# HpWang-whu/RoReg

Hardware: AMD Instinct MI355X
Metric: pair-registrations/sec (higher is better)
Workload: dtype f32 (every f32 operand enters the fp16 matrix cores as hi + lo fp16 under a per-keypoint power-of-two block scale: <= 22 significant bits relative to a CONSERVATIVE per-keypoint bound -- measured on the extractor: the bound sits 2^2..2^6 above the keypoint's true coefficient maximum (config.f16x2_sc

## Files before the change

### include/roreg_hip.h

```cpp
#ifndef ROREG_HIP_H
#define ROREG_HIP_H

#include <stdint.h>
#include <stddef.h>

#ifdef __cplusplus
extern "C" {
#endif

#define ROREG_ABI_VERSION 6
int roreg_abi_version(void);
const char *roreg_last_error(void);

int roreg_set_group_tables(const int32_t *P_host, const int32_t *Nei_host, const double *R_host);

size_t roreg_group_conv_packed_size(int Cin, int Cout, int KS);
int roreg_group_conv_pack_weights(const float *W_host , int Cin, int Cout, int KS,
                                  float *wpack_host );
size_t roreg_group_conv_workspace_size(int B, int Cin, int Cout, int Lin, int Lout, int KS);
int roreg_group_conv(const float *x, const float *wpack, const float *bias,
                     const float *bn_scale, const float *bn_shift, const float *residual,
                     float *out, const int32_t *gather,
                     int B, int Cin, int Cout, int Lin, int Lout, int KS,
                     float *workspace, size_t workspace_floats, void *stream);

int roreg_group_conv_split(const float *x, const void *wsplit, const float *bias, const float *bn_scale, const float *bn_shift,
                           float *out, const int32_t *gather,
                           const int32_t *lds_order , int lds_stride,
                           int B, int Cin, int Cout, int Lin, int Lout, int KS, void *stream);

int roreg_dense_split(const float *x, const void *wsplit, const float *bias, const float *scale, const float *shift,
                      const float *residual, int residual_stride, float *out, int B, int K, int O, void *stream);

int roreg_group_conv_f16x2(const float *x, const void *wsplit2, int w_exp, const float *bias, const float *bn_scale, const float *bn_shift,
                           float act_smax, float act_tmax, const float *in_rowmax_dev, float *out, float *out_rowmax_dev,
                           const int32_t *gather, const int32_t *lds_order , int lds_stride,
                           int B, int Cin, int Cout, int Lin, int Lout, int KS, void *stream);
int roreg_dense_f16x2(const float *x, const void *wsplit2, int w_exp, const float *bias, const float *scale, const float *shift,
                      float act_smax, float act_tmax, const float *in_rowmax_dev, const float *residual, int residual_stride, float *out,
                      float *out_rowmax_dev, int B, int K, int O, void *stream);
int roreg_group_conv_f16x2_packed(const uint32_t *x_words, const void *wsplit2, int w_exp, const float *bias, const float *in_bound_dev,
                                  float *out, float *out_rowmax_dev, const int32_t *gather, const int32_t *lds_order, int lds_stride,
                                  int B, int Cin, int Cout, int Lin, int Lout, int KS, void *stream);

int roreg_gf_finalize(const float *eqv_raw, void *eqv, int eqv_bf16 ,
                      float *inv, int B, void *stream);

int roreg_det_score(const float *enc, float *scores, int B, void *stream);

int roreg_inv_descriptor(const void *eqv, int eqv_bf16 , float *inv, int N,
                         void *stream);

int roreg_nn_search(const float *src, const int64_t *src_rows, int m,
                    const float *tgt, const int64_t *tgt_rows, int n, int F,
                    int64_t *idx_out, float *dist_out, uint64_t *scratch, void *stream);

int roreg_nn_search_ex(const float *src, const int64_t *src_rows, int m,
                       const float *tgt, const int64_t *tgt_rows, int n, int F, int squared,
                       int64_t *idx_out, float *dist_out, uint64_t *scratch, void *stream);

int roreg_pdist(const float *A, int m, const float *B, int n, int F, int squared, float *out, void *stream);

typedef struct {
    const float *desc0, *desc1;
    const int64_t *rows0, *rows1;
    int32_t m0, m1;
} roreg_match_task;
size_t roreg_mutual_match_batch_workspace(int n_tasks, int max_m);
int roreg_mutual_match_batch(const roreg_match_task *tasks_dev, int n_tasks, int max_m, int64_t *match_out, int32_t *counts_out,
                             void *workspace, size_t workspace_bytes, void *stream);

size_t roreg_knn_search_workspace(int m, int n);
int roreg_knn_search(const float *src, int m, const float *tgt, int n, int F, int k,
                     int64_t *idx_out, void *workspace , size_t workspace_bytes, void *stream);

int roreg_knn_search_ex(const float *src, int m, const float *tgt, int n, int F, int k, int squared, int64_t *idx_out, float *dist_out,
                        void *workspace, size_t workspace_bytes, void *stream);

size_t roreg_knn_search_seg_workspace(long long m_total, int n_seg, int max_m, int max_n);
int roreg_knn_search_seg(const float *src, const float *tgt, const int32_t *seg_src, const int32_t *seg_tgt, int n_seg, long long m_total,
                         int max_m, int max_n, int F, int k, int64_t *idx_out, void *workspace, size_t workspace_bytes, void *stream);

int roreg_mutual_matches(const int64_t *nn01, const int64_t *nn10, int m, int n ,
                         const int64_t *sample0, const int64_t *sample1,
                         int64_t *match_out, int32_t *count_out, void *stream);

int roreg_des2r(const float *feats1, const int64_t *rows1, const float *feats0, const int64_t *rows0,
                int M, int64_t *idx_out, float *cor_out, void *stream);

int roreg_group_corr(const float *perm_feats, const int64_t *perm_rows, const float *bcast_feats, const int64_t *bcast_rows,
                     int M, int transpose_table, int64_t *idx_out, float *cor_out, void *stream);

int roreg_group_corr_mfma(const float *perm_feats, const int64_t *perm_rows, const float *bcast_feats, const int64_t *bcast_rows, int M,
                          int transpose_table, float *cor_out, void *stream);

int roreg_set_des2r_tables(int transpose_table , const uint8_t *ia_host,
                           const uint8_t *ib_host, const uint8_t *cnt_host, const float *NT_host);
int roreg_group_corr_irrep(const float *perm_coefs, const int64_t *perm_rows, const float *bcast_coefs, const int64_t *bcast_rows, int M,
                           int transpose_table, float *cor_out, void *stream);
int roreg_des2r_irrep(const float *coef1, const int64_t *rows1, const float *coef0, const int64_t *rows0, const void *feats1,
                      const void *feats0, int feat_bf16, int M, int64_t *idx_out, void *stream);
int roreg_des2r_recheck_count(int reset, int32_t *count_out);
int roreg_feat_coefs(const void *x, int x_bf16, float *out, int B, int C, int split, void *stream);

int roreg_et_gather(const void *before0, const void *before1, const void *after0, const void *after1,
                    int feat_bf16 ,
                    const int64_t *rows0, const int64_t *rows1, const int64_t *pre_idx, int M,
                    float *x_out, void *stream);

int roreg_quat_to_trans(const float *q, const int64_t *anchor, const double *keys0, const int64_t *rows0,
                        const double *keys1, const int64_t *rows1, int M,
                        double *Trans_out, float *quat_out, void *stream);

int roreg_ransac_score(const double *k0, const double *k1, const double *w, int w_f32, int M,
                       const double *Trans, const int64_t *hyp_rows, int H, double ird,
                       double *overlap_out, int32_t *best_out, uint8_t *mask_out, void *stream);

int roreg_refine(const double *k0, const double *k1, const double *w, int w_f32, int M,
                 const double *T_in, int t_in_stride ,
                 const double *Trans, const int64_t *hyp_rows, const int32_t *best,
                 double dist, double *T_out, double *stats_out ,
                 void *stream);

typedef struct {
    const void *before0, *before1, *after0, *after1;
    const double *keys0, *keys1;
    const int64_t *matches;
    const int64_t *sel;
    int32_t n, pad_;
    int64_t off;
    const float *coef0, *coef1;
} roreg_lt_task;
int roreg_lt_prepare_batch(const roreg_lt_task *tasks_dev, int n_tasks, int max_n, int flags, int64_t *dr_out, float *x_out,
                           const float *bn_scale , const float *bn_shift, float *x_bound_out , void *stream);
int roreg_lt_finish_batch(const roreg_lt_task *tasks_dev, int n_tasks, int max_n, const float *q_all, const int64_t *dr_all,
                          double *Trans_out, void *stream);
int roreg_role_max(const void *before, const void *after, int feat_bf16, const float *bn_scale , const float *bn_shift, float *out,
                   int N, void *stream);
int roreg_row_bound_roles(const void *x_spatial, int x_bf16, float *bound_out, const float *role_scale, const float *role_shift, float *role_out, int B,
                          void *stream);
int roreg_inv_descriptor_roles(const void *eqv, int eqv_bf16, float *inv, const float *role_scale, const float *role_shift, float *role_out, int N,
                               void *stream);
int roreg_lt_prepare_rows(const roreg_lt_task *tasks_dev, const float *const *roles_dev, int n_tasks, int max_n, int flags, int64_t *dr_out,
                          uint64_t *rows_out, float *x_bound_out, void *stream);

typedef struct {
    const double *keys0, *keys1;
    const int64_t *matches;
    const double *w;
    const double *Trans;
    const int64_t *hyp_rows;
    int32_t M, H;
    int64_t koff;
// ... 258 lines not shown
```

### roreg_amd/_abi.py

```python
import ctypes
from ctypes import c_int, c_void_p, c_size_t, c_double, c_float, c_char_p

import numpy as np

ABI_VERSION = 6

_P = c_void_p
PROTOTYPES = {
    'roreg_abi_version': (c_int, []),
    'roreg_last_error': (c_char_p, []),
    'roreg_set_group_tables': (c_int, [_P, _P, _P]),
    'roreg_group_conv_packed_size': (c_size_t, [c_int, c_int, c_int]),
    'roreg_group_conv_pack_weights': (c_int, [_P, c_int, c_int, c_int, _P]),
    'roreg_group_conv_workspace_size': (c_size_t, [c_int, c_int, c_int, c_int, c_int, c_int]),
    'roreg_group_conv': (c_int, [_P, _P, _P, _P, _P, _P, _P, _P, c_int, c_int, c_int, c_int, c_int, c_int, _P, c_size_t, _P]),
    'roreg_group_conv_split': (c_int, [_P, _P, _P, _P, _P, _P, _P, _P, c_int, c_int, c_int, c_int, c_int, c_int, c_int, _P]),
    'roreg_group_conv_f16x2': (c_int, [_P, _P, c_int, _P, _P, _P, c_float, c_float, _P, _P, _P, _P, _P, c_int, c_int, c_int, c_int, c_int, c_int, c_int, _P]),
    'roreg_group_conv_f16x2_packed': (c_int, [_P, _P, c_int, _P, _P, _P, _P, _P, _P, c_int, c_int, c_int, c_int, c_int, c_int, c_int, _P]),
    'roreg_dense_f16x2': (c_int, [_P, _P, c_int, _P, _P, _P, c_float, c_float, _P, _P, c_int, _P, _P, c_int, c_int, c_int, _P]),
    'roreg_dense_split': (c_int, [_P, _P, _P, _P, _P, _P, c_int, _P, c_int, c_int, c_int, _P]),
    'roreg_gf_finalize': (c_int, [_P, _P, c_int, _P, c_int, _P]),
    'roreg_det_score': (c_int, [_P, _P, c_int, _P]),
    'roreg_inv_descriptor': (c_int, [_P, c_int, _P, c_int, _P]),
    'roreg_nn_search': (c_int, [_P, _P, c_int, _P, _P, c_int, c_int, _P, _P, _P, _P]),
    'roreg_nn_search_ex': (c_int, [_P, _P, c_int, _P, _P, c_int, c_int, c_int, _P, _P, _P, _P]),
    'roreg_pdist': (c_int, [_P, c_int, _P, c_int, c_int, c_int, _P, _P]),
    'roreg_knn_search_workspace': (c_size_t, [c_int, c_int]),
    'roreg_knn_search': (c_int, [_P, c_int, _P, c_int, c_int, c_int, _P, _P, c_size_t, _P]),
    'roreg_knn_search_ex': (c_int, [_P, c_int, _P, c_int, c_int, c_int, c_int, _P, _P, _P, c_size_t, _P]),
    'roreg_knn_search_seg_workspace': (c_size_t, [ctypes.c_longlong, c_int, c_int, c_int]),
    'roreg_knn_search_seg': (c_int, [_P, _P, _P, _P, c_int, ctypes.c_longlong, c_int, c_int, c_int, c_int, _P, _P, c_size_t, _P]),
    'roreg_mutual_matches': (c_int, [_P, _P, c_int, c_int, _P, _P, _P, _P, _P]),
    'roreg_mutual_match_batch_workspace': (c_size_t, [c_int, c_int]),
    'roreg_mutual_match_batch': (c_int, [_P, c_int, c_int, _P, _P, _P, c_size_t, _P]),
    'roreg_des2r': (c_int, [_P, _P, _P, _P, c_int, _P, _P, _P]),
    'roreg_set_des2r_tables': (c_int, [c_int, _P, _P, _P, _P]),
    'roreg_group_corr_irrep': (c_int, [_P, _P, _P, _P, c_int, c_int, _P, _P]),
    'roreg_group_corr_mfma': (c_int, [_P, _P, _P, _P, c_int, c_int, _P, _P]),
    'roreg_des2r_irrep': (c_int, [_P, _P, _P, _P, _P, _P, c_int, c_int, _P, _P]),
    'roreg_des2r_recheck_count': (c_int, [c_int, _P]),
    'roreg_feat_coefs': (c_int, [_P, c_int, _P, c_int, c_int, c_int, _P]),
    'roreg_et_gather': (c_int, [_P, _P, _P, _P, c_int, _P, _P, _P, c_int, _P, _P]),
    'roreg_quat_to_trans': (c_int, [_P, _P, _P, _P, _P, _P, c_int, _P, _P, _P]),
    'roreg_ransac_score': (c_int, [_P, _P, _P, c_int, c_int, _P, _P, c_int, c_double, _P, _P, _P, _P]),
    'roreg_refine': (c_int, [_P, _P, _P, c_int, c_int, _P, c_int, _P, _P, _P, c_double, _P, _P, _P]),
    'roreg_lt_prepare_batch': (c_int, [_P, c_int, c_int, c_int, _P, _P, _P, _P, _P, _P]),
    'roreg_lt_finish_batch': (c_int, [_P, c_int, c_int, _P, _P, _P, _P]),
    'roreg_role_max': (c_int, [_P, _P, c_int, _P, _P, _P, c_int, _P]),
    'roreg_row_bound_roles': (c_int, [_P, c_int, _P, _P, _P, _P, c_int, _P]),
    'roreg_inv_descriptor_roles': (c_int, [_P, c_int, _P, _P, _P, _P, c_int, _P]),
    'roreg_lt_prepare_rows': (c_int, [_P, _P, c_int, c_int, c_int, _P, _P, _P, _P]),
    'roreg_ransac_batch_workspace': (c_size_t, [c_int, ctypes.c_longlong, c_int]),
    'roreg_ransac_batch': (c_int, [_P, c_int, ctypes.c_longlong, c_int, c_int, c_double, c_int, _P, _P, _P, _P, _P, _P, c_size_t, _P]),
    'roreg_refine_batch': (c_int, [_P, _P, c_int, ctypes.c_longlong, _P, ctypes.c_double, c_int, _P, _P, _P, _P]),
    'roreg_yohoc_draw': (c_int, [_P, ctypes.c_longlong, _P, _P, c_int, c_int, _P, _P, _P, _P]),
    'roreg_gather_rows_batch': (c_int, [_P, c_int, c_int, c_int, _P]),
    'roreg_gather_rows_f64': (c_int, [_P, _P, c_int, c_int, _P, _P]),
    'roreg_group_corr': (c_int, [_P, _P, _P, _P, c_int, c_int, _P, _P, _P]),
    'roreg_topk_dot_workspace_size': (c_size_t, [c_int, c_int, c_int]),
    'roreg_topk_dot': (c_int, [_P, c_int, _P, c_int, c_int, _P, _P, _P, c_size_t, _P, _P, c_int, c_int, c_int, _P]),
    'roreg_context_colmax': (c_int, [_P, c_int, _P, c_int, c_int, _P, _P, _P]),
    'roreg_sinkhorn_batch_workspace_size': (c_size_t, [c_int, c_int, c_int, ctypes.c_longlong, ctypes.c_longlong]),
    'roreg_sinkhorn_batch_consts': (c_int, [_P, _P, c_int, _P]),
    'roreg_sinkhorn_batch': (c_int, [_P, _P, _P, _P, _P, _P, _P, c_int, c_float, c_int, _P, _P, _P, _P, _P, c_size_t, _P]),
    'roreg_sinkhorn_batch2_workspace_size': (c_size_t, [c_int, c_int, c_int, ctypes.c_longlong, ctypes.c_longlong]),
    'roreg_sinkhorn_batch2': (c_int, [_P, _P, _P, _P, _P, _P, _P, c_int, c_float, c_int, _P, _P, _P, _P, _P, c_size_t, c_int, _P]),
    'roreg_sinkhorn_batch3_workspace_size': (c_size_t, [c_int, c_int, c_int, ctypes.c_longlong, ctypes.c_longlong, c_int, c_int]),
    'roreg_sinkhorn_batch3': (c_int, [_P, _P, _P, _P, _P, _P, _P, c_int, c_float, c_int, _P, _P, _P, _P, _P, c_size_t, c_int, _P, _P]),
    'roreg_write_files': (c_int, [_P, _P, _P, _P, _P, c_int, c_int]),
    'roreg_yohoc_draw_many': (c_int, [_P, c_int, _P, _P, c_int, c_int, _P, _P, _P, c_int]),
    'roreg_mlp_head_workspace': (c_size_t, [c_int, c_int, c_int]),
    'roreg_mlp_head': (c_int, [_P, _P, _P, _P, _P, c_int, c_int, c_int, c_int, _P, _P, c_int, _P, _P, _P, _P, _P, c_int, c_int, c_float, _P, _P, _P]),
    'roreg_sinkhorn_early_exit': (c_int, [c_int]),
    'roreg_sinkhorn_iteration_stats': (c_int, [_P, _P, c_int, _P]),
    'roreg_linear': (c_int, [_P, c_int, c_int, _P, _P, c_int, _P, _P]),
    'roreg_linear_mfma': (c_int, [_P, c_int, c_int, _P, _P, c_int, _P, _P]),
    'roreg_linear_path': (c_int, [c_int]),
    'roreg_linear_cat3': (c_int, [_P, _P, _P, _P, c_int, c_int, _P, _P, c_int, _P, _P]),
    'roreg_gemm_persistent': (c_int, [c_int]),
    'roreg_gemm_thin': (c_int, [c_int]),
    'roreg_gf_finish_route': (c_int, [c_int]),
    'roreg_irrep_gemm_f16x2_rows': (c_int, [_P, _P, _P, _P, c_int, c_int, c_int, _P]),
    'roreg_gf_finish': (c_int, [_P, _P, _P, _P, _P, _P, _P, _P, _P, c_int, _P]),
    'roreg_instnorm_stats': (c_int, [_P, c_int, c_int, c_float, _P, _P, _P, c_int, c_int, _P]),
    'roreg_mlp_tail': (c_int, [_P, c_int, c_int, _P, _P, _P, _P, _P, c_int, c_int, _P]),
    'roreg_mlp_tail_mfma': (c_int, [_P, c_int, c_int, _P, _P, _P, _P, _P, c_int, c_int, _P]),
    'roreg_knn_attention': (c_int, [_P, _P, _P, _P, c_int, c_int, c_int, c_int, _P, _P]),
    'roreg_rm_elementwise': (c_int, [c_int, _P, _P, _P, _P, c_int, c_int, c_int, _P, _P, _P]),
    'roreg_sinkhorn_workspace_size': (c_size_t, [c_int, c_int]),
    'roreg_sinkhorn': (c_int, [_P, c_int, _P, c_int, c_float, c_int, _P, _P, _P, _P, _P, _P, c_size_t, _P]),
    'roreg_icp_grid_size': (c_size_t, [_P, _P, c_int, c_double, _P, _P]),
    'roreg_icp_grid_build': (c_int, [_P, _P, _P, _P, c_size_t, _P]),
    'roreg_icp_batch_workspace': (c_size_t, [c_int, ctypes.c_longlong]),
    'roreg_icp_batch': (c_int, [_P, c_int, _P, c_int, ctypes.c_longlong, c_double, c_int, c_double, c_double, _P, _P, _P, _P, _P, _P, _P, _P, c_size_t, _P]),
    'roreg_icp_normals': (c_int, [_P, c_double, c_int, _P, _P]),
    'roreg_icp_plane_batch_workspace': (c_size_t, [c_int, ctypes.c_longlong]),
    'roreg_icp_plane_batch': (c_int, [_P, c_int, _P, c_int, ctypes.c_longlong, c_double, c_int, c_double, c_double, _P, _P, _P, _P, _P, _P, _P, _P, c_size_t, _P]),
    'roreg_icp_gicp_batch_workspace': (c_size_t, [c_int, ctypes.c_longlong]),
    'roreg_icp_gicp_batch': (c_int, [_P, c_int, _P, c_int, ctypes.c_longlong, c_double, c_int, c_double, c_double, _P, _P, _P, _P, _P, _P, _P, _P, c_size_t, _P]),
    'roreg_icp_eval_workspace': (c_size_t, [c_int, ctypes.c_longlong]),
    'roreg_icp_eval_batch': (c_int, [_P, c_int, _P, c_int, ctypes.c_longlong, c_double, _P, _P, _P, _P, _P, c_size_t, _P]),
    'roreg_voxel_workspace': (c_size_t, [c_int]),
    'roreg_voxel_downsample': (c_int, [_P, c_int, c_double, _P, _P, _P, _P, _P, _P, _P, c_size_t, _P]),
    'roreg_pg_workspace': (c_size_t, [_P, c_int]),
    'roreg_pg_optimize_batch': (c_int, [_P, _P, c_int, _P, _P, _P, _P, _P, _P, _P, _P, _P, _P, _P, c_int, c_int, _P, _P, _P, _P, _P, _P, _P, _P, _P, _P, _P, c_size_t, _P]),
    'roreg_sparse_map_workspace': (c_size_t, [c_int]),
    'roreg_sparse_stride_map': (c_int, [_P, c_int, c_int, _P, c_int, _P, _P, _P, _P, _P, c_size_t, _P]),
    'roreg_sparse_kernel_map': (c_int, [_P, c_int, _P, c_int, c_int, c_int, _P, _P, _P, c_size_t, _P]),
    'roreg_sparse_conv': (c_int, [_P, c_int, c_int, c_int, _P, c_int, c_int, _P, c_int, _P, _P, _P, c_int, c_int, _P, c_int, _P]),
    'roreg_sparse_l2norm': (c_int, [_P, c_int, c_int, _P, _P]),
    'roreg_group_feature_assemble': (c_int, [_P, c_int, c_int, _P, _P, c_int, c_int, c_int, _P, c_int, _P, _P]),
    'roreg_sc2_workspace': (c_size_t, [ctypes.c_longlong, ctypes.c_longlong, ctypes.c_longlong, _P]),
    'roreg_sc2_hypotheses_batch': (c_int, [_P, c_int, ctypes.c_longlong, ctypes.c_longlong, ctypes.c_longlong, c_int, c_int, c_double, c_int, _P, _P, _P, _P, c_size_t, _P]),
    'roreg_fpfh_spfh_workspace': (c_size_t, [c_int]),
    'roreg_fpfh_features_workspace': (c_size_t, [c_int]),
    'roreg_fpfh_orient': (c_int, [_P, c_int, _P, _P, _P, _P]),
    'roreg_fpfh_spfh': (c_int, [_P, c_int, _P, c_double, _P, _P, _P, c_size_t, _P]),
# ... 53 lines not shown
```

### roreg_amd/csrc/mfma_match.hip

```cpp
#include "common.h"
#include "primitives.h"

#pragma clang fp contract(off)

namespace {

struct MatchTask {
    const float *desc0, *desc1;
    const int64_t *rows0, *rows1;
    int32_t m0, m1;
};

constexpr int F = 32, TILE = 128, LP = 36;
constexpr float PAD_NORM = 1e30f;

struct WS {
    float *G;
    float *N;
    unsigned *AM;
    unsigned long long *PK;
    unsigned *MX;
};
__host__ __device__ inline size_t ws_task_bytes(int P) { return (size_t)2 * P * (F * 4 + 4 + 4 + 8) + 64; }
__device__ __forceinline__ WS ws_of(char *base, int task, int P) {
    char *p = base + (size_t)task * ws_task_bytes(P);
    WS w;
    w.PK = reinterpret_cast<unsigned long long *>(p); p += (size_t)2 * P * 8;
    w.G = reinterpret_cast<float *>(p); p += (size_t)2 * P * F * 4;
    w.N = reinterpret_cast<float *>(p); p += (size_t)2 * P * 4;
    w.AM = reinterpret_cast<unsigned *>(p); p += (size_t)2 * P * 4;
    w.MX = reinterpret_cast<unsigned *>(p);
    return w;
}

__device__ __forceinline__ unsigned f2o(float x) { const unsigned b = __float_as_uint(x); return b ^ ((b >> 31) ? 0xffffffffu : 0x80000000u); }
__device__ __forceinline__ float o2f(unsigned k) { return __uint_as_float(k ^ ((k >> 31) ? 0x80000000u : 0xffffffffu)); }

__global__ __launch_bounds__(256) void mm_prepare_kernel(const MatchTask *__restrict__ tasks, int P, char *__restrict__ wsb) {
    const int task = blockIdx.z >> 1, side = blockIdx.z & 1;
    const MatchTask t = tasks[task];
    const WS w = ws_of(wsb, task, P);
    const float *desc = side ? t.desc1 : t.desc0;
    const int64_t *rows = side ? t.rows1 : t.rows0;
    const int m = side ? t.m1 : t.m0;
    const int j = blockIdx.x * 8 + (threadIdx.x >> 5), f = threadIdx.x & 31;
    if (blockIdx.x == 0 && threadIdx.x == 0) w.MX[side] = 0u;
    if (j >= P) return;
    float v = 0.f;
    if (j < m) v = desc[(size_t)(rows ? rows[j] : (int64_t)j) * F + f];
    w.G[((size_t)side * P + j) * F + f] = v;
    float s = v * v;
#pragma unroll
    for (int o = 16; o > 0; o >>= 1) s += __shfl_xor(s, o);
    if (f == 0) {
        w.N[(size_t)side * P + j] = j < m ? s : PAD_NORM;
        w.AM[(size_t)side * P + j] = 0xffffffffu;
        w.PK[(size_t)side * P + j] = ~0ull;
    }
}

__global__ __launch_bounds__(256) void mm_maxnorm_kernel(const MatchTask *__restrict__ tasks, int P, char *__restrict__ wsb) {
    const int task = blockIdx.z >> 1, side = blockIdx.z & 1;
    const MatchTask t = tasks[task];
    const WS w = ws_of(wsb, task, P);
    const int m = side ? t.m1 : t.m0;
    const int j = blockIdx.x * 256 + threadIdx.x;
    float v = (j < m) ? w.N[(size_t)side * P + j] : 0.f;
#pragma unroll
    for (int o = 32; o > 0; o >>= 1) v = fmaxf(v, __shfl_xor(v, o));
    if ((threadIdx.x & 63) == 0 && v > 0.f) atomicMax(&w.MX[side], __float_as_uint(v));
}

__device__ __forceinline__ int norm_exp(float n2) {
    if (!(n2 > 0.f) || !(n2 < __builtin_inff())) return 0;
    int ex;
    (void)frexpf(n2, &ex);
    return 14 - ((ex + 1) >> 1);
}
__device__ __forceinline__ float exact_dist(const float *__restrict__ s, const float *__restrict__ t) {
    float acc = 0.f;
#pragma unroll
    for (int f = 0; f < F; ++f) {
        const float d = __fsub_rn(s[f], t[f]);
        acc = __fadd_rn(acc, __fmul_rn(d, d));
// ... 219 lines not shown
        float cnext = 0.f;
        if (jt + 1 < ntj) {
            dma_tile(w.G + ((size_t)P + j0 + TILE) * F, Tb + (buf ^ 1) * TP);
            cnext = load_consts(jt + 1);
        }
        f32x16 c[2][2];
#pragma unroll
        for (int a = 0; a < 2; ++a)
#pragma unroll
            for (int b = 0; b < 2; ++b)
#pragma unroll
                for (int r = 0; r < 16; ++r) c[a][b][r] = 0.f;
#pragma unroll
        for (int st = 0; st < 2; ++st) {
            f16x8 tf[2][2];
#pragma unroll
            for (int g = 0; g < 2; ++g) {
                const int rt = wn * 64 + g * 32 + jl;
                const float4 v0 = *reinterpret_cast<const float4 *>(T + swz_piece(rt, st * 4 + h * 2) * 4);
                const float4 v1 = *reinterpret_cast<const float4 *>(T + swz_piece(rt, st * 4 + h * 2 + 1) * 4);
                const float x8[8] = {v0.x, v0.y, v0.z, v0.w, v1.x, v1.y, v1.z, v1.w};
                split2(x8, xs1[buf * TILE + rt], tf[g][0], tf[g][1]);
            }
#pragma unroll
            for (int a = 0; a < 2; ++a)
#pragma unroll
                for (int b = 0; b < 2; ++b) c[a][b] = split_mma<2>(sf[st][a], tf[b], c[a][b]);
        }
#pragma unroll
        for (int b = 0; b < 2; ++b) {
            const int jc = wn * 64 + b * 32 + jl;
            const float nj = n1s[buf * TILE + jc], isj = is1[buf * TILE + jc];
            if constexpr (!VERIFY) {
                float mn = __builtin_inff();
#pragma unroll
                for (int a = 0; a < 2; ++a)
#pragma unroll
                    for (int r = 0; r < 16; ++r) {
                        const int ir = cd_row32(r, h, wm * 64 + a * 32);
                        const float av = (n0s[ir] + nj) - 2.f * ((c[a][b][r] * is0[ir]) * isj);
                        mn = fminf(mn, av);
                        rmin[a][r] = fminf(rmin[a][r], av);
                    }
                mn = fminf(mn, __shfl_xor(mn, 32));
                if (h == 0) atomicMin(cm + j0 + jc, f2o(mn));
            } else {
                const float tj = thr1[buf * TILE + jc] + (1e-4f * (nj + mx0) + 1e-6f);
                unsigned m0 = 0u, m1 = 0u;
#pragma unroll
                for (int a = 0; a < 2; ++a)
#pragma unroll
                    for (int r = 0; r < 16; ++r) {
                        const int ir = cd_row32(r, h, wm * 64 + a * 32);
                        const float av = (n0s[ir] + nj) - 2.f * ((c[a][b][r] * is0[ir]) * isj);
                        m0 |= (av <= thr0[ir] ? 1u : 0u) << (a * 16 + r);
                        m1 |= (av <= tj ? 1u : 0u) << (a * 16 + r);
                    }
                unsigned m = m0 | m1;
                while (m) {
                    const int q = __ffs(m) - 1;
                    m &= m - 1;
                    const int ir = cd_row32(q & 15, h, wm * 64 + (q >> 4) * 32);
                    const float d = exact_dist_swz(S, ir, T, jc);
                    const unsigned long long db = (unsigned long long)__float_as_uint(d) << 32;
                    if (((m0 >> q) & 1u) && j0 + jc < t.m1) atomicMin(&w.PK[i0 + ir], db | (unsigned)(j0 + jc));
                    if (((m1 >> q) & 1u) && i0 + ir < t.m0) atomicMin(&w.PK[(size_t)P + j0 + jc], db | (unsigned)(i0 + ir));
                }
            }
        }
        if (jt + 1 < ntj) store_consts(buf ^ 1, cnext);
        asm volatile("s_waitcnt vmcnt(0) lgkmcnt(0)" ::: "memory");
        __syncthreads();
    }
    if constexpr (!VERIFY) {
#pragma unroll
        for (int a = 0; a < 2; ++a)
#pragma unroll
            for (int r = 0; r < 16; ++r) {
                float v = rmin[a][r];
#pragma unroll
                for (int o = 16; o > 0; o >>= 1) v = fminf(v, __shfl_xor(v, o));
                const int ir = cd_row32(r, h, wm * 64 + a * 32);
                if (jl == 0 && i0 + ir < t.m0) atomicMin(&w.AM[i0 + ir], f2o(v));
            }
        for (int j = tid; j < t.m1; j += 256) atomicMin(&w.AM[(size_t)P + j], cm[j]);
    }
}

__global__ __launch_bounds__(1024) void mm_mutual_kernel(const MatchTask *__restrict__ tasks, int P, char *__restrict__ wsb, int out_pitch,
                                                         int64_t *__restrict__ match_all, int32_t *__restrict__ counts) {
    __shared__ int wave_cnt[16];
    __shared__ int base;
    const int task = blockIdx.x;
    const MatchTask t = tasks[task];
    const WS w = ws_of(wsb, task, P);
    const unsigned long long *p01 = w.PK, *p10 = w.PK + P;
    int64_t *match_out = match_all + (size_t)task * out_pitch * 2;
    const int m = t.m1 > 0 ? t.m0 : 0;
    const int tid = threadIdx.x, lane = tid & 63, wv = tid >> 6;
    if (tid == 0) base = 0;
    __syncthreads();
    for (int start = 0; start < m; start += 1024) {
        const int i = start + tid;
        bool keep = false;
        int64_t j = 0;
        if (i < m) {
            j = (int64_t)(p01[i] & 0xffffffffu);
            keep = j < (int64_t)t.m1 && (int64_t)(p10[j] & 0xffffffffu) == (int64_t)i;
        }
        const unsigned long long mask = __ballot(keep);
        const int before = __popcll(mask & ((1ull << lane) - 1ull));
        if (lane == 0) wave_cnt[wv] = __popcll(mask);
        __syncthreads();
        int woff = 0, total = 0;
#pragma unroll
        for (int q = 0; q < 16; ++q) {
            const int cq = wave_cnt[q];
            if (q < wv) woff += cq;
            total += cq;
        }
        const int b0 = base;
        if (keep) {
            const int pos = b0 + woff + before;
            match_out[2 * pos] = t.rows0 ? t.rows0[i] : (int64_t)i;
            match_out[2 * pos + 1] = t.rows1 ? t.rows1[j] : j;
        }
        __syncthreads();
        if (tid == 0) base = b0 + total;
        __syncthreads();
    }
    if (tid == 0) counts[task] = base;
}

}

extern "C" size_t roreg_mutual_match_batch_workspace(int n_tasks, int max_m) {
    const int P = (max_m + TILE - 1) / TILE * TILE;
    return (size_t)n_tasks * ws_task_bytes(P > 0 ? P : TILE);
}

extern "C" int roreg_mutual_match_batch(const roreg_match_task *tasks_dev, int n_tasks, int max_m, int64_t *match_out, int32_t *counts_out,
                                        void *workspace, size_t workspace_bytes, void *stream) {
    if (n_tasks == 0) return 0;
    ROREG_REQUIRE(tasks_dev && match_out && counts_out && workspace && n_tasks > 0 && max_m >= 0, "roreg_mutual_match_batch: bad arguments");
    ROREG_REQUIRE(workspace_bytes >= roreg_mutual_match_batch_workspace(n_tasks, max_m), "roreg_mutual_match_batch: workspace too small");
    ROREG_REQUIRE(n_tasks <= 65535, "roreg_mutual_match_batch: too many tasks in one call (%d)", n_tasks);
    static_assert(sizeof(roreg_match_task) == sizeof(MatchTask), "roreg_match_task layout");
    hipStream_t s = roreg::as_stream(stream);
    const MatchTask *tasks = reinterpret_cast<const MatchTask *>(tasks_dev);
    const int P = max_m > 0 ? (max_m + TILE - 1) / TILE * TILE : TILE;
    char *ws = reinterpret_cast<char *>(workspace);
    const int out_pitch = (max_m + 1) & ~1;
    if (max_m > 0) {
        hipLaunchKernelGGL(mm_prepare_kernel, dim3(P / 8, 1, 2 * n_tasks), dim3(256), 0, s, tasks, P, ws);
        hipLaunchKernelGGL(mm_maxnorm_kernel, dim3(P / 256 + 1, 1, 2 * n_tasks), dim3(256), 0, s, tasks, P, ws);
        const dim3 grid(P / TILE, P / TILE, n_tasks);
        roreg::ProfScope prof(roreg::PROF_MM_TILE, s);
        static const bool bf16x3 = [] { const char *e = getenv("ROREG_MATCH_BF16X3"); return e && e[0] == '1'; }();
        static const bool tiles = [] { const char *e = getenv("ROREG_MATCH_TILES"); return e && e[0] == '1'; }();
        const size_t lds_strip = (size_t)(3 * TP + 12 * TILE) * 4 + (size_t)P * 4;
        if (!bf16x3 && !tiles && lds_strip <= 80 * 1024) {
            const dim3 sgrid(P / TILE, n_tasks);
            if (roreg::launch_lds("roreg_mutual_match_batch", mm_strip_kernel<false>, sgrid, dim3(256), lds_strip, s, tasks, P, ws) ||
                roreg::launch_lds("roreg_mutual_match_batch", mm_strip_kernel<true>, sgrid, dim3(256), lds_strip, s, tasks, P, ws)) return 1;
        } else if (bf16x3) {
            hipLaunchKernelGGL((mm_tile_kernel<false, 3>), grid, dim3(256), 0, s, tasks, P, ws);
            hipLaunchKernelGGL((mm_tile_kernel<true, 3>), grid, dim3(256), 0, s, tasks, P, ws);
        } else {
            hipLaunchKernelGGL((mm_tile_kernel<false, 2>), grid, dim3(256), 0, s, tasks, P, ws);
            hipLaunchKernelGGL((mm_tile_kernel<true, 2>), grid, dim3(256), 0, s, tasks, P, ws);
        }
    }
    hipLaunchKernelGGL(mm_mutual_kernel, dim3(n_tasks), dim3(1024), 0, s, tasks, P, ws, out_pitch, match_out, counts_out);
    ROREG_CHECK_LAUNCH("roreg_mutual_match_batch");
    return 0;
}
```

### roreg_amd/hip.py

```python
import ctypes
import os
import threading
from ctypes import c_int, c_void_p, c_size_t, c_double, c_float, c_char_p

import numpy as np
import torch

from .group import tables

_LIB_PATH = os.environ.get('ROREG_HIP_LIB') or os.path.join(os.path.dirname(os.path.abspath(__file__)), 'libroreg_hip.so')

GEMM_MODES = ('f16x2', 'bf16x3', 'f32')
GEMM_MODE = os.environ.get('ROREG_GEMM', 'f16x2')
if GEMM_MODE == 'split':
    GEMM_MODE = 'bf16x3'
if GEMM_MODE not in GEMM_MODES:
    raise ValueError(f"ROREG_GEMM must be one of {GEMM_MODES}, got {GEMM_MODE!r}")
XDMA = os.environ.get('ROREG_GEMM_XDMA', '1') == '1'
MFMA16 = os.environ.get('ROREG_GEMM_MFMA16', '1') == '1'


def use_planes(O):
    return bool(XDMA and O % 256 == 0 and not os.environ.get('ROREG_TILE_M128'))
_lib = None
# ... 615 lines not shown
    rows = np.empty((n, max(max_iter, 1), 3), np.int64); n_hyp = np.empty(n, np.int32); giveup = np.zeros((n, 4, 4), np.float64)
    if n:
        nt = n_threads if n_threads is not None else max(1, min(32, (os.cpu_count() or 2) // 2, n // 8 + 1))
        _check(lib().roreg_yohoc_draw_many(c_void_p(seeds.ctypes.data), n, c_void_p(flat.ctypes.data), c_void_p(offs.ctypes.data), int(max_iter), int(max_tries),
                                           c_void_p(rows.ctypes.data), c_void_p(n_hyp.ctypes.data), c_void_p(giveup.ctypes.data), int(nt)), 'roreg_yohoc_draw_many')
    return [None if n_hyp[p] < 0 else rows[p, :n_hyp[p]] for p in range(n)], giveup


def ransac_batch(tasks, ird, w_f32=False, keep=False):
    n = len(tasks)
    dev = tasks[0][0].device if n else torch.device('cuda')
    best = torch.empty(n, dtype=torch.int32, device=dev)
    T1 = torch.empty((n, 4, 4), dtype=torch.float64, device=dev); T2 = torch.empty_like(T1)
    st1 = torch.empty((n, 16), dtype=torch.float64, device=dev); st2 = torch.empty_like(st1)
    if n == 0:
        return (best, T1, st1, T2, st2, None) if keep else (best, T1, st1, T2, st2)
    table = np.zeros(n, _RANSAC_TASK)
    koff = 0
    for i, (k0, k1, m, w, Tr, hr) in enumerate(tasks):
        _ptr(k0, torch.float64); _ptr(k1, torch.float64); _ptr(m, torch.int64); _ptr(Tr, torch.float64)
        if w is not None:
            _ptr(w, torch.float64)
        if hr is not None:
            _ptr(hr, torch.int64)
        M = int(m.shape[0]); H = int(hr.shape[0]) if hr is not None else int(Tr.shape[0])
        table[i] = (k0.data_ptr(), k1.data_ptr(), m.data_ptr() if M else 0, w.data_ptr() if w is not None else 0, Tr.data_ptr() if H else 0,
                    hr.data_ptr() if hr is not None else 0, M, H, koff)
        koff += M
    max_M = int(table['M'].max()); max_H = int(table['H'].max())
    tdev = upload(table.view(np.uint8).reshape(n, _RANSAC_TASK.itemsize))
    ws_n = lib().roreg_ransac_batch_workspace(n, koff, max_H)
    ws = torch.empty(max(ws_n, 8) // 8, dtype=torch.float64, device=dev)
    _check(lib().roreg_ransac_batch(_ptr(tdev), n, koff, max(max_M, 1), max_H, float(ird), int(bool(w_f32)), _ptr(best), _ptr(T1), _ptr(st1), _ptr(T2), _ptr(st2),
                                    _ptr(ws), ws_n, _stream()), 'roreg_ransac_batch')
    if keep:
        return best, T1, st1, T2, st2, (tdev, ws, koff, bool(w_f32), tasks)
    return best, T1, st1, T2, st2


def refine_batch(ctx, sel, T_in, dist):
    tdev, ws, total_M, w_f32, _tasks = ctx
    n = len(sel)
    dev = ws.device
    T = torch.empty((n, 4, 4), dtype=torch.float64, device=dev); st = torch.empty((n, 16), dtype=torch.float64, device=dev)
    if n == 0:
        return T, st
    sel_dev = upload(np.ascontiguousarray(sel, np.int32))
    Tin = T_in if torch.is_tensor(T_in) else upload(np.ascontiguousarray(T_in, np.float64))
    _check(lib().roreg_refine_batch(_ptr(tdev), _ptr(sel_dev, torch.int32), n, total_M, _ptr(Tin, torch.float64), float(dist), int(w_f32), _ptr(T), _ptr(st),
                                    _ptr(ws), _stream()), 'roreg_refine_batch')
    return T, st




def mutual_match_batch(tasks):
    n = len(tasks)
    table = np.zeros(n, _MATCH_TASK)
    keep = []
    for i, (d0, d1, r0, r1) in enumerate(tasks):
        if d0.shape[1] != 32 or d1.shape[1] != 32:
            raise HipError('mutual_match_batch: descriptors must be [*,32] float32')
        for t in (d0, d1):
            _ptr(t, torch.float32)
        table[i] = (d0.data_ptr(), d1.data_ptr(), r0.data_ptr() if r0 is not None else 0, r1.data_ptr() if r1 is not None else 0,
                    r0.shape[0] if r0 is not None else d0.shape[0], r1.shape[0] if r1 is not None else d1.shape[0])
        for t in (r0, r1):
            if t is not None:
                _ptr(t, torch.int64)
    dev = tasks[0][0].device if n else torch.device('cuda')
    max_m = int(max([0] + [max(int(t['m0']), int(t['m1'])) for t in table]))
    pitch = (max_m + 1) & ~1
    out = torch.empty((n, max(pitch, 1), 2), dtype=torch.int64, device=dev)
    cnt = torch.zeros(max(n, 1), dtype=torch.int32, device=dev)[:n]
    if n == 0:
        return out, cnt
    tdev = upload(table.view(np.uint8).reshape(n, _MATCH_TASK.itemsize))
    ws_n = lib().roreg_mutual_match_batch_workspace(n, max_m)
    ws = torch.empty(max(ws_n, 8) // 8, dtype=torch.int64, device=dev)
    _check(lib().roreg_mutual_match_batch(_ptr(tdev), n, max_m, _ptr(out), _ptr(cnt), _ptr(ws), ws_n, _stream()), 'roreg_mutual_match_batch')
    return out, cnt


_des2r_ready = False


def des2r_tables(transpose=False):
    from .fourier import group_fourier, DIMS
    gf = group_fourier(); T = tables()
    ia = np.zeros((60, 5), np.uint8); ib = np.zeros((60, 5), np.uint8); cnt = np.zeros(60, np.uint8)
    NT = np.zeros((60, 60), np.float64)
    for q, (ri, i, j) in enumerate(gf.index):
        d = DIMS[ri]; off = int(gf.offsets[ri])
        cnt[q] = d
        for k in range(5):
            kk = min(k, d - 1)
            if not transpose:
                ia[q, k] = off + i * d + kk; ib[q, k] = off + j * d + kk
            else:
                ia[q, k] = off + kk * d + j; ib[q, k] = off + kk * d + i
        NT[q, :] = gf.rho[ri][:, j, i]
    rng = np.random.default_rng(0)
    d1 = rng.standard_normal((4, 60)); d2 = rng.standard_normal((4, 60))
    perm = (lambda a: T.P[:, a]) if transpose else (lambda a: T.P[a])
    want = np.array([(d1[:, perm(a)] * d2).sum() for a in range(60)])
    X1 = d1 @ gf.F.T; X2 = d2 @ gf.F.T
    C = np.array([sum((X2[f, ia[q, :cnt[q]]] * X1[f, ib[q, :cnt[q]]]).sum() for f in range(4)) for q in range(60)])
    assert np.abs(C @ NT - want).max() < 1e-11, 'irrep-domain correlation identity violated'
    return ia, ib, cnt, np.ascontiguousarray(NT, np.float32)


def ensure_des2r():
    global _des2r_ready
    if not _des2r_ready:
        ensure_tables(); ensure_fourier()
        for mode in (0, 1):
            ia, ib, cnt, NT = des2r_tables(transpose=bool(mode))
            _check(lib().roreg_set_des2r_tables(mode, ia.ctypes.data, ib.ctypes.data, cnt.ctypes.data, NT.ctypes.data), 'roreg_set_des2r_tables')
        _des2r_ready = True


def feat_coefs(x):
    ensure_fourier()
    B, C = int(x.shape[0]), int(x.shape[1])
    out = torch.empty((B, C, 60), dtype=torch.float32, device=x.device)
    xp, bf = _feat(x)
    _check(lib().roreg_feat_coefs(xp, bf, _ptr(out), B, C, {'f16x2': 2, 'bf16x3': 1, 'f32': 0}[GEMM_MODE], _stream()), 'roreg_feat_coefs')
    return out


def des2r_recheck_count(reset=True):
    ensure_des2r()
    n = ctypes.c_int32(0)
    _check(lib().roreg_des2r_recheck_count(1 if reset else 0, ctypes.byref(n)), 'roreg_des2r_recheck_count')
    return n.value


def des2r(feats1, feats0, rows1=None, rows0=None, want_cor=False, coefs1=None, coefs0=None):
    ensure_tables()
    M = int(rows1.shape[0]) if rows1 is not None else int(feats1.shape[0])
    if coefs1 is not None and not want_cor:
        ensure_des2r()
        idx = torch.empty(M, dtype=torch.int64, device=feats1.device)
        p1, bf1 = _feat(feats1); p0, bf0 = _feat(feats0)
        if bf1 != bf0:
            raise HipError('des2r: feats1 and feats0 must share one dtype')
        _check(lib().roreg_des2r_irrep(_ptr(coefs1, torch.float32), _ptr(rows1, torch.int64), _ptr(coefs0, torch.float32), _ptr(rows0, torch.int64),
                                       p1, p0, bf1, M, _ptr(idx), _stream()), 'roreg_des2r_irrep')
        return idx
    idx = torch.empty(M, dtype=torch.int64, device=feats1.device)
    cor = torch.empty((M, 60), dtype=torch.float32, device=feats1.device) if want_cor else None
    _check(lib().roreg_des2r(_ptr(feats1, torch.float32), _ptr(rows1, torch.int64), _ptr(feats0, torch.float32), _ptr(rows0, torch.int64),
                             M, _ptr(idx), _ptr(cor), _stream()), 'roreg_des2r')
    return (idx, cor) if want_cor else idx


def et_gather(before0, before1, after0, after1, pre_idx, rows0=None, rows1=None, out=None):
    ensure_tables()
    M = pre_idx.shape[0]
    x = out if out is not None else torch.empty((M, 128, 60), dtype=torch.float32, device=before0.device)
    assert x.shape == (M, 128, 60)
    ptrs = [_feat(t) for t in (before0, before1, after0, after1)]
    if len({f for _, f in ptrs}) != 1:
        raise HipError('et_gather: the four feature tensors must share one dtype')
    _check(lib().roreg_et_gather(ptrs[0][0], ptrs[1][0], ptrs[2][0], ptrs[3][0], ptrs[0][1], _ptr(rows0, torch.int64), _ptr(rows1, torch.int64),
                                 _ptr(pre_idx, torch.int64), M, _ptr(x), _stream()), 'roreg_et_gather')
# ... 122 lines not shown
```

Baseline: 1141.

## Add register-resident strip mutual-match kernel and make it the default

Adds a variant of the strip mutual-match kernel that keeps the source tile's fp16 hi/lo fragments and per-row constants (norms, scales, thresholds) in registers across all target tiles, so they are no longer reloaded and re-split from LDS each iteration. It also tracks the per-row running minimum in registers, prefetches the next tile's constants, and batches candidate-queue draining to every 16 tiles. A runtime switch (environment variable plus a C ABI setter and a Python context manager) selects between old and new forms, with the new one on by default. The cost is higher register pressure under launch_bounds(256,2), which could reduce occupancy or cause spills.

```diff
diff --git a/include/roreg_hip.h b/include/roreg_hip.h
--- a/include/roreg_hip.h
+++ b/include/roreg_hip.h
@@ -69,6 +69,7 @@
 size_t roreg_mutual_match_batch_workspace(int n_tasks, int max_m);
 int roreg_mutual_match_batch(const roreg_match_task *tasks_dev, int n_tasks, int max_m, int64_t *match_out, int32_t *counts_out,
                              void *workspace, size_t workspace_bytes, void *stream);
+int roreg_match_form(int form);
 
 size_t roreg_knn_search_workspace(int m, int n);
 int roreg_knn_search(const float *src, int m, const float *tgt, int n, int F, int k,
diff --git a/roreg_amd/_abi.py b/roreg_amd/_abi.py
--- a/roreg_amd/_abi.py
+++ b/roreg_amd/_abi.py
@@ -33,6 +33,7 @@
     'roreg_mutual_matches': (c_int, [_P, _P, c_int, c_int, _P, _P, _P, _P, _P]),
     'roreg_mutual_match_batch_workspace': (c_size_t, [c_int, c_int]),
     'roreg_mutual_match_batch': (c_int, [_P, c_int, c_int, _P, _P, _P, c_size_t, _P]),
+    'roreg_match_form': (c_int, [c_int]),
     'roreg_des2r': (c_int, [_P, _P, _P, _P, c_int, _P, _P, _P]),
     'roreg_set_des2r_tables': (c_int, [c_int, _P, _P, _P, _P]),
     'roreg_group_corr_irrep': (c_int, [_P, _P, _P, _P, c_int, c_int, _P, _P]),
diff --git a/roreg_amd/csrc/mfma_match.hip b/roreg_amd/csrc/mfma_match.hip
--- a/roreg_amd/csrc/mfma_match.hip
+++ b/roreg_amd/csrc/mfma_match.hip
@@ -1,5 +1,6 @@
 #include "common.h"
 #include "primitives.h"
+#include <atomic>
 
 #pragma clang fp contract(off)
 
@@ -385,6 +386,209 @@
                 for (int o = 16; o > 0; o >>= 1) v = fminf(v, __shfl_xor(v, o));
                 const int ir = cd_row32(r, h, wm * 64 + a * 32);
                 if (jl == 0 && i0 + ir < t.m0) atomicMin(&w.AM[i0 + ir], f2o(v));
+            }
+        for (int j = tid; j < t.m1; j += 256) atomicMin(&w.AM[(size_t)P + j], cm[j]);
+    }
+}
+
+template <bool VERIFY>
+__global__ __launch_bounds__(256, 2) void mm_strip_regs_kernel(const MatchTask *__restrict__ tasks, int P, char *__restrict__ wsb) {
+    extern __shared__ __attribute__((aligned(16))) char smem[];
+    float *S = reinterpret_cast<float *>(smem);
+    float *Tb = S + TP;
+    float *n0s = Tb + 2 * TP, *xs0 = n0s + TILE, *is0 = xs0 + TILE, *thr0 = is0 + TILE;
+    float *n1s = thr0 + TILE, *xs1 = n1s + 2 * TILE, *is1 = xs1 + 2 * TILE, *thr1 = is1 + 2 * TILE;
+    unsigned *cm = reinterpret_cast<unsigned *>(thr1 + 2 * TILE);
+    unsigned *cq = cm;
+    const int qcap = P - 1;
+    const int task = blockIdx.y;
+    const MatchTask t = tasks[task];
+    const int i0 = blockIdx.x * TILE;
+    if (i0 >= t.m0 || t.m1 <= 0) return;
+    const WS w = ws_of(wsb, task, P);
+    const int tid = threadIdx.x, lane = tid & 63, wv = tid >> 6;
+    const int wm = wv & 1, wn = wv >> 1, jl = lane & 31, h = lane >> 5;
+    const int ntj = (t.m1 + TILE - 1) / TILE;
+    const float mx0 = VERIFY ? __uint_as_float(w.MX[0]) : 0.f, mx1 = VERIFY ? __uint_as_float(w.MX[1]) : 0.f;
+
+    auto dma_tile = [&](const float *src, float *dst) {
+#pragma unroll
+        for (int k = 0; k < 4; ++k) {
+            const int q = k * 256 + tid, row = q >> 3, cs = q & 7;
+            __builtin_amdgcn_global_load_lds((const __attribute__((address_space(1))) void *)(src + swz_piece(row, cs) * 4),
+                                             (__attribute__((address_space(3))) void *)(dst + (k * 256 + wv * 64) * 4), 16, 0, 0);
+        }
+    };
+    auto load_consts = [&](int jt) -> float {
+        const int r = tid & (TILE - 1);
+        if (tid < TILE) return w.N[(size_t)P + jt * TILE + r];
+        return VERIFY ? o2f(w.AM[(size_t)P + jt * TILE + r]) : 0.f;
+    };
+    auto drain_queue = [&]() {
+        const int n = min((int)cq[0], qcap);
+        for (int e = tid; e < n; e += 256) {
+            const unsigned en = cq[1 + e];
+            const int ir = en & 127, j = (en >> 7) & 8191;
+            const float4 *tp = reinterpret_cast<const float4 *>(w.G + ((size_t)P + j) * F);
+            float tv[F];
+#pragma unroll
+            for (int p = 0; p < F / 4; ++p) { const float4 v = tp[p]; tv[4 * p] = v.x; tv[4 * p + 1] = v.y; tv[4 * p + 2] = v.z; tv[4 * p + 3] = v.w; }
+            float acc = 0.f;
+#pragma unroll
+            for (int f = 0; f < F; ++f) {
+                const float d = __fsub_rn(S[swz_piece(ir, f >> 2) * 4 + (f & 3)], tv[f]);
+                acc = __fadd_rn(acc, __fmul_rn(d, d));
+            }
+            const float d = sqrtf(__fadd_rn(acc, 1e-7f));
+            const unsigned long long db = (unsigned long long)__float_as_uint(d) << 32;
+            if (((en >> 20) & 1u) && j < t.m1) atomicMin(&w.PK[i0 + ir], db | (unsigned)j);
+            if (((en >> 21) & 1u) && i0 + ir < t.m0) atomicMin(&w.PK[(size_t)P + j], db | (unsigned)(i0 + ir));
+        }
+        __syncthreads();
+        if (tid == 0) cq[0] = 0u;
+        __syncthreads();
+    };
+    auto store_consts = [&](int buf, float v) {
+        const int r = tid & (TILE - 1);
+        if (tid < TILE) {
+            const int e = norm_exp(v);
+            n1s[buf * TILE + r] = v; xs1[buf * TILE + r] = ldexpf(1.f, e); is1[buf * TILE + r] = ldexpf(1.f, -e);
+        } else if (VERIFY) thr1[buf * TILE + r] = v;
+    };
+
+    dma_tile(w.G + (size_t)i0 * F, S);
+    dma_tile(w.G + (size_t)P * F, Tb);
+    {
+        const float c0 = load_consts(0);
+        if (tid < TILE) {
+            const float a = w.N[i0 + tid];
+            const int e = norm_exp(a);
+            n0s[tid] = a; xs0[tid] = ldexpf(1.f, e); is0[tid] = ldexpf(1.f, -e);
+            if (VERIFY) thr0[tid] = (o2f(w.AM[i0 + tid]) - a) + (1e-4f * (a + mx1) + 1e-6f);
+        }
+        store_consts(0, c0);
+        if (!VERIFY)
+            for (int j = tid; j < P; j += 256) cm[j] = 0xffffffffu;
+        else if (tid == 0) cq[0] = 0u;
+    }
+    asm volatile("s_waitcnt vmcnt(0) lgkmcnt(0)" ::: "memory");
+    __syncthreads();
+
+    f16x8 sf[2][2][2];
+#pragma unroll
+    for (int st = 0; st < 2; ++st)
+#pragma unroll
+        for (int g = 0; g < 2; ++g) {
+            const int rs = wm * 64 + g * 32 + jl;
+            const float4 u0 = *reinterpret_cast<const float4 *>(S + swz_piece(rs, st * 4 + h * 2) * 4);
+            const float4 u1 = *reinterpret_cast<const float4 *>(S + swz_piece(rs, st * 4 + h * 2 + 1) * 4);
+            const float x8[8] = {u0.x, u0.y, u0.z, u0.w, u1.x, u1.y, u1.z, u1.w};
+            split2(x8, xs0[rs], sf[st][g][0], sf[st][g][1]);
+        }
+    float m2is0[2][16], n0r[2][16], third[2][16];
+#pragma unroll
+    for (int a = 0; a < 2; ++a)
+#pragma unroll
+        for (int r = 0; r < 16; ++r) {
+            const int ir = cd_row32(r, h, wm * 64 + a * 32);
+            m2is0[a][r] = -2.f * is0[ir]; n0r[a][r] = n0s[ir]; third[a][r] = VERIFY ? thr0[ir] : __builtin_inff();
+        }
+
+    for (int jt = 0; jt < ntj; ++jt) {
+        const int buf = jt & 1, j0 = jt * TILE;
+        const float *T = Tb + buf * TP;
+        float cnext = 0.f;
+        if (jt + 1 < ntj) {
+            dma_tile(w.G + ((size_t)P + j0 + TILE) * F, Tb + (buf ^ 1) * TP);
+            cnext = load_consts(jt + 1);
+        }
+#pragma unroll
+        for (int b = 0; b < 2; ++b) {
+            const int jc = wn * 64 + b * 32 + jl;
+            f32x16 c[2];
+#pragma unroll
+            for (int a = 0; a < 2; ++a)
+#pragma unroll
+                for (int r = 0; r < 16; ++r) c[a][r] = 0.f;
+#pragma unroll
+            for (int st = 0; st < 2; ++st) {
+                f16x8 tf[2];
+                const float4 v0 = *reinterpret_cast<const float4 *>(T + swz_piece(jc, st * 4 + h * 2) * 4);
+                const float4 v1 = *reinterpret_cast<const float4 *>(T + swz_piece(jc, st * 4 + h * 2 + 1) * 4);
+                const float x8[8] = {v0.x, v0.y, v0.z, v0.w, v1.x, v1.y, v1.z, v1.w};
+                split2(x8, xs1[buf * TILE + jc], tf[0], tf[1]);
+#pragma unroll
+                for (int a = 0; a < 2; ++a) c[a] = split_mma<2>(sf[st][a], tf, c[a]);
+            }
+            const float nj = n1s[buf * TILE + jc], isj = is1[buf * TILE + jc];
+            if constexpr (!VERIFY) {
+                float mn = __builtin_inff();
+#pragma unroll
+                for (int r = 0; r < 16; ++r) {
+                    const float u0 = __builtin_fmaf(c[0][r] * isj, m2is0[0][r], nj), u1 = __builtin_fmaf(c[1][r] * isj, m2is0[1][r], nj);
+                    third[0][r] = fminf(third[0][r], u0); third[1][r] = fminf(third[1][r], u1);
+                    mn = fminf(fminf(mn, u0 + n0r[0][r]), u1 + n0r[1][r]);
+                }
+                mn = fminf(mn, __shfl_xor(mn, 32));
+                if (h == 0) atomicMin(cm + j0 + jc, f2o(mn));
+            } else {
+                const float tj = thr1[buf * TILE + jc] + (1e-4f * (nj + mx0) + 1e-6f);
+                unsigned m0 = 0u, m1 = 0u;
+#pragma unroll
+                for (int a = 0; a < 2; ++a)
+#pragma unroll
+                    for (int r4 = 0; r4 < 16; r4 += 4) {
+                        float u[4];
+                        unsigned long long any = 0ull;
+#pragma unroll
+                        for (int q = 0; q < 4; ++q) {
+                            u[q] = __builtin_fmaf(c[a][r4 + q] * isj, m2is0[a][r4 + q], nj);
+                            any |= __builtin_amdgcn_ballot_w64(u[q] <= third[a][r4 + q]) | __builtin_amdgcn_ballot_w64(u[q] + n0r[a][r4 + q] <= tj);
+                        }
+                        if (any) {
+#pragma unroll
+                            for (int q = 0; q < 4; ++q) {
+                                m0 |= (u[q] <= third[a][r4 + q] ? 1u : 0u) << (a * 16 + r4 + q);
+                                m1 |= (u[q] + n0r[a][r4 + q] <= tj ? 1u : 0u) << (a * 16 + r4 + q);
+                            }
+                        }
+                    }
+                unsigned m = m0 | m1;
+                if (m) {
+                    unsigned slot = atomicAdd(cq, (unsigned)__popc(m));
+                    while (m) {
+                        const int q = __ffs(m) - 1;
+                        m &= m - 1;
+                        const int ir = cd_row32(q & 15, h, wm * 64 + (q >> 4) * 32);
+                        const unsigned k0 = (m0 >> q) & 1u, k1 = (m1 >> q) & 1u;
+                        if (slot < (unsigned)qcap) cq[1 + slot] = (unsigned)ir | (unsigned)(j0 + jc) << 7 | k0 << 20 | k1 << 21;
+                        else {
+                            const float d = exact_dist_swz(S, ir, T, jc);
+                            const unsigned long long db = (unsigned long long)__float_as_uint(d) << 32;
+                            if (k0 && j0 + jc < t.m1) atomicMin(&w.PK[i0 + ir], db | (unsigned)(j0 + jc));
+                            if (k1 && i0 + ir < t.m0) atomicMin(&w.PK[(size_t)P + j0 + jc], db | (unsigned)(i0 + ir));
+                        }
+                        ++slot;
+                    }
+                }
+            }
+        }
+        if (jt + 1 < ntj) store_consts(buf ^ 1, cnext);
+        asm volatile("s_waitcnt vmcnt(0) lgkmcnt(0)" ::: "memory");
+        __syncthreads();
+        if constexpr (VERIFY)
+            if ((jt & 15) == 15 || jt + 1 == ntj) drain_queue();
+    }
+    if constexpr (!VERIFY) {
+#pragma unroll
+        for (int a = 0; a < 2; ++a)
+#pragma unroll
+            for (int r = 0; r < 16; ++r) {
+                float v = third[a][r];
+#pragma unroll
+                for (int o = 16; o > 0; o >>= 1) v = fminf(v, __shfl_xor(v, o));
+                const int ir = cd_row32(r, h, wm * 64 + a * 32);
+                if (jl == 0 && i0 + ir < t.m0) atomicMin(&w.AM[i0 + ir], f2o(v + n0r[a][r]));
             }
         for (int j = tid; j < t.m1; j += 256) atomicMin(&w.AM[(size_t)P + j], cm[j]);
     }
@@ -435,7 +639,28 @@
     if (tid == 0) counts[task] = base;
 }
 
-}
+struct MatchSwitch {
+    std::atomic<int> v{-1};
+    int get() {
+        int x = v.load(std::memory_order_relaxed);
+        if (x < 0) {
+            const char *e = getenv("ROREG_MATCH_FORM");
+            x = e && (e[0] == '0' || e[0] == '1') ? e[0] - '0' : 1;
+            v.store(x, std::memory_order_relaxed);
+        }
+        return x;
+    }
+    int set(int form) {
+        const int prev = get();
+        if (form == 0 || form == 1) v.store(form, std::memory_order_relaxed);
+        return prev;
+    }
+};
+MatchSwitch g_match_form;
+
+}
+
+extern "C" int roreg_match_form(int form) { return g_match_form.set(form); }
 
 extern "C" size_t roreg_mutual_match_batch_workspace(int n_tasks, int max_m) {
     const int P = (max_m + TILE - 1) / TILE * TILE;
@@ -464,8 +689,11 @@
         const size_t lds_strip = (size_t)(3 * TP + 12 * TILE) * 4 + (size_t)P * 4;
         if (!bf16x3 && !tiles && lds_strip <= 80 * 1024) {
             const dim3 sgrid(P / TILE, n_tasks);
-            if (roreg::launch_lds("roreg_mutual_match_batch", mm_strip_kernel<false>, sgrid, dim3(256), lds_strip, s, tasks, P, ws) ||
-                roreg::launch_lds("roreg_mutual_match_batch", mm_strip_kernel<true>, sgrid, dim3(256), lds_strip, s, tasks, P, ws)) return 1;
+            if (g_match_form.get() == 0) {
+                if (roreg::launch_lds("roreg_mutual_match_batch", mm_strip_kernel<false>, sgrid, dim3(256), lds_strip, s, tasks, P, ws) ||
+                    roreg::launch_lds("roreg_mutual_match_batch", mm_strip_kernel<true>, sgrid, dim3(256), lds_strip, s, tasks, P, ws)) return 1;
+            } else if (roreg::launch_lds("roreg_mutual_match_batch", mm_strip_regs_kernel<false>, sgrid, dim3(256), lds_strip, s, tasks, P, ws) ||
+                       roreg::launch_lds("roreg_mutual_match_batch", mm_strip_regs_kernel<true>, sgrid, dim3(256), lds_strip, s, tasks, P, ws)) return 1;
         } else if (bf16x3) {
             hipLaunchKernelGGL((mm_tile_kernel<false, 3>), grid, dim3(256), 0, s, tasks, P, ws);
             hipLaunchKernelGGL((mm_tile_kernel<true, 3>), grid, dim3(256), 0, s, tasks, P, ws);
diff --git a/roreg_amd/hip.py b/roreg_amd/hip.py
--- a/roreg_amd/hip.py
+++ b/roreg_amd/hip.py
@@ -721,6 +721,19 @@
     return out, cnt
 
 
+class match_form:
+
+    def __init__(self, form=1):
+        self.form = int(form)
+
+    def __enter__(self):
+        self.prev = lib().roreg_match_form(self.form)
+
+    def __exit__(self, *exc):
+        lib().roreg_match_form(self.prev)
+        return False
+
+
 _des2r_ready = False
 
 
```

Measured after the change: 1149 (median of 6 runs). Within noise of the previous version (+0.6%).
